# SebastianAment/CovarianceFunctions.jl

Hardware: AMD Instinct MI355X
Metric: Gramian MVMs/sec, dense EQ kernel, n=131072, d=3, fp32 (+ achieved HBM GB/s in roofline.hbm_*) (higher is better)
Workload: dtype f32; 1 GPU; EQ dense Gramian mul!, d=3 n=131072 fp32 (BASELINE.json configs[1]); x ~ N(0, I_3), a ~ N(0,1), alpha=1, beta=0, y == x; all n*m entries evaluated; points/a/b resident in HBM; n=131072, d=3, kernel=EQ, parallelism=1 GPU

## Files before the change

covariancefunctions.jl_amd/covgram/_ffi.py:

```python
from __future__ import annotations

import ctypes as C
import os

_HERE = os.path.dirname(os.path.abspath(__file__))
LIB_PATH = os.environ.get("COVGRAM_LIB") or os.path.normpath(os.path.join(_HERE, "..", "lib", "libcovgram.so"))

EQ, EXP, RQ, GAMMAEXP, CAUCHY, IMQ, MATERNP, DOT, EXPDOT, MATERN, ASINDOT = range(11)
CONSTANT, COMPOSITE = 100, 101
COMPOSITE_MAX_TERMS, COMPOSITE_MAX_FACTORS = 8, 8
ISOTROPIC, DOTPRODUCT = 1, 2
F32, F64 = 0, 1
HOST, DEVICE = 0, 1
OK, EINVAL, EUNSUPPORTED, EHIP, ENODEVICE, ENOMEM = 0, -1, -2, -3, -4, -5
MATERNP_MAX_P = 8
PIVCHOL_MAX_RANK = 1024
SM_MAX_COMPONENTS, SM_MAX_D = 32, 16
BILINEAR_MAX_NVEC, BILINEAR_MAX_D = 32, 64
COMM_ID_BYTES = 128
BCG_SLAB, BCG_FIELDS = 64, 8
BCG_RZ, BCG_TOL2, BCG_RR, BCG_ACTIVE, BCG_ITERS = range(5)
BLOCK_GRADIENT, BLOCK_VALUE_GRADIENT, BLOCK_HESSIAN, BLOCK_VALUE_GRADIENT_HESSIAN = range(4)
ABI_VERSION = 113

# ... 31 lines not shown

class DimensionMismatch(CovgramError, ValueError):
    """Julia's DimensionMismatch (src/util.jl:41, :9) — raised for COVGRAM_EINVAL."""


class UnsupportedKernel(CovgramError, NotImplementedError):
    """Kernel / dimension outside the compiled device set (COVGRAM_EUNSUPPORTED)."""


class NoDevice(CovgramError):
    """No gfx950 device: the product path fails loudly (COVGRAM_ENODEVICE)."""


_P = C.c_void_p
_I64 = C.c_int64
_I32 = C.c_int32
_D = C.c_double
_KP = C.POINTER(covgram_kernel)

PROTOTYPES = {
    "covgram_version": (C.c_int, []),
    "covgram_sizeof_kernel": (C.c_int, []),
    "covgram_sizeof_composite": (C.c_int, []),
    "covgram_last_error": (C.c_char_p, []),
    "covgram_device_count": (C.c_int, [C.POINTER(C.c_int)]),
    "covgram_ctx_create": (C.c_int, [C.POINTER(_P), C.c_int, _P]),
    "covgram_ctx_destroy": (C.c_int, [_P]),
    "covgram_ctx_set_stream": (C.c_int, [_P, _P]),
    "covgram_ctx_get_stream": (C.c_int, [_P, C.POINTER(_P)]),
    "covgram_ctx_set_option": (C.c_int, [_P, C.c_char_p, _I64]),
    "covgram_ctx_get_info": (C.c_int, [_P, C.c_char_p, C.POINTER(_I64)]),
    "covgram_sync": (C.c_int, [_P]),
    "covgram_ctx_kernel_time": (C.c_int, [_P, C.POINTER(_D), C.POINTER(_I64), _I32]),
    "covgram_points_create": (C.c_int, [_P, C.POINTER(_P), _P, _I64, _I32, _I32, _I32]),
    "covgram_points_slice": (C.c_int, [_P, _I64, _I64, C.POINTER(_P)]),
    "covgram_points_destroy": (C.c_int, [_P]),
    "covgram_points_info": (C.c_int, [_P, C.POINTER(_I64), C.POINTER(_I32), C.POINTER(_I32)]),
    "covgram_mvm": (C.c_int, [_P, _KP, _P, _P, _P, _I64, _P, _I64, _I32, _D, _D, _I32]),
    "covgram_matrix": (C.c_int, [_P, _KP, _P, _P, _P, _I64, _I32]),
    "covgram_grad_mvm": (C.c_int, [_P, _KP, _P, _P, _P, _I64, _P, _I64, _I32, _D, _D, _I32]),
    "covgram_valgrad_mvm": (C.c_int, [_P, _KP, _P, _P, _P, _I64, _P, _I64, _I32, _D, _D, _I32]),
    "covgram_hess_mvm": (C.c_int, [_P, _KP, _P, _P, _P, _I64, _P, _I64, _I32, _D, _D, _I32]),
    "covgram_valgradhess_mvm": (C.c_int, [_P, _KP, _P, _P, _P, _I64, _P, _I64, _I32, _D, _D, _I32]),
    "covgram_block_matrix": (C.c_int, [_P, _I32, _KP, _P, _P, _P, _I64, _I32]),
    "covgram_mvm_sym_supported": (C.c_int, [_P, _KP, _P, _I32, C.POINTER(C.c_int32)]),
    "covgram_mvm_sym_partial": (C.c_int, [_P, _KP, _P, _P, _P, _I32, _I32]),
    "covgram_comm_unique_id": (C.c_int, [_P, _I64]),
    "covgram_comm_create": (C.c_int, [_P, _P, _I32, _I32]),
    "covgram_comm_destroy": (C.c_int, [_P]),
    "covgram_comm_info": (C.c_int, [_P, C.POINTER(_I32), C.POINTER(_I32)]),
    "covgram_comm_all_gather": (C.c_int, [_P, _P, _P, _I64, _I32]),
    "covgram_comm_all_reduce_sum": (C.c_int, [_P, _P, _I64, _I32]),
    "covgram_mvm_sharded": (C.c_int, [_P, _KP, _P, _P, _P, _P, _D, _D]),
    "covgram_mvm_sym_allreduce": (C.c_int, [_P, _KP, _P, _P, _P, _D, _D]),
    "covgram_decay_radius": (C.c_int, [_KP, _D, C.POINTER(_D)]),
    "covgram_sparse_create": (C.c_int, [_P, C.POINTER(_P), _KP, _P, _P, _D]),
    "covgram_sparse_info": (C.c_int, [_P, C.POINTER(_I64), C.POINTER(_I64), C.POINTER(_I64), C.POINTER(_I32), C.POINTER(_D)]),
    "covgram_sparse_export": (C.c_int, [_P, _P, _P, _P, _I32]),
    "covgram_sparse_mvm": (C.c_int, [_P, _P, _I64, _P, _I64, _I32, _D, _D, _I32]),
    "covgram_sparse_destroy": (C.c_int, [_P]),
    "covgram_bh_create": (C.c_int, [_P, C.POINTER(_P), _KP, _P, _P, _D, _I32]),
    "covgram_bh_info": (C.c_int, [_P, C.POINTER(_I64), C.POINTER(_I64), C.POINTER(_I32), C.POINTER(_I32), C.POINTER(_I64), C.POINTER(_I32),
                                  C.POINTER(_D)]),
    "covgram_bh_export": (C.c_int, [_P, _P, _P, _P, _P, _P, _P, _P, _I32]),
    "covgram_bh_moments": (C.c_int, [_P, _P, _P, _P, _I32]),
    "covgram_bh_mvm": (C.c_int, [_P, _P, _P, _D, _D, _D, _I32, _P, _I64, _I32]),
# ... 64 lines not shown
```

covariancefunctions.jl_amd/csrc/api.hip:

```cpp
#include <math.h>
#include <stdarg.h>

#include <algorithm>
#include <vector>

#include "driver.hpp"
#include "dense_mvm.hpp"
#include "dense_sym32.hpp"
#include "dense_bcast.hpp"
#include "dense_wide.hpp"
#include "grad_wide.hpp"
#include "hess_mvm.hpp"
#include "block_matrix.hpp"

namespace covgram {

static thread_local char g_err[512] = "";

void set_error(const char* fmt, ...) {
    va_list ap;
    va_start(ap, fmt);
    vsnprintf(g_err, sizeof(g_err), fmt, ap);
    va_end(ap);
}
// ... 577 lines not shown
    ::covgram::DeviceGuard _cg_dev(ctx->device);
    (void)hipStreamSynchronize(ctx->stream);
    ctx_blas_destroy(ctx);
    (void)comm_destroy(ctx);
    for (auto& w : ctx->ws) if (w.ptr) (void)hipFree(w.ptr);
    if (ctx->sym_map) (void)hipFree(ctx->sym_map);
    if (ctx->stamp_buf) (void)hipFree(ctx->stamp_buf);
    if (ctx->tickets) (void)hipFree(ctx->tickets);
    for (auto& t : ctx->timers) { (void)hipEventDestroy(t.first); (void)hipEventDestroy(t.second); }
    if (ctx->own_stream) (void)hipStreamDestroy(ctx->stream);
    delete ctx;
    return COVGRAM_OK;
}

int covgram_ctx_set_stream(covgram_ctx* ctx, void* hip_stream) {
    CG_REQUIRE(ctx != nullptr, COVGRAM_EINVAL, "ctx is NULL");
    if ((hipStream_t)hip_stream != ctx->stream) CG_CHECK_HIP(hipStreamSynchronize(ctx->stream));
    ctx->stream = (hipStream_t)hip_stream;
    return COVGRAM_OK;
}

int covgram_ctx_get_stream(covgram_ctx* ctx, void** hip_stream) {
    CG_REQUIRE(ctx && hip_stream, COVGRAM_EINVAL, "NULL argument");
    *hip_stream = (void*)ctx->stream;
    return COVGRAM_OK;
}

struct CtxField { const char* key; int64_t covgram_ctx::*member; };
#define CG_FIELD(name) {#name, &covgram_ctx::name}
static const CtxField kOptions[] = {
    CG_FIELD(dense_variant), CG_FIELD(toeplitz_fused), CG_FIELD(toeplitz_colfft), CG_FIELD(toeplitz_persist), CG_FIELD(kron_fill), CG_FIELD(mfma_f16),
    CG_FIELD(mfma_gate_pct), CG_FIELD(mfma_fuse_w), CG_FIELD(toeplitz_real_spectrum), CG_FIELD(rows_per_lane), CG_FIELD(jsplit), CG_FIELD(target_wgs),
    CG_FIELD(grad_keep_r), CG_FIELD(grad_expand), CG_FIELD(grad_bcast), CG_FIELD(mfma_lds), CG_FIELD(mfma_sym), CG_FIELD(dense_sym), CG_FIELD(dense_bcast),
    CG_FIELD(mfma_stamp), CG_FIELD(inkernel_reduce), CG_FIELD(matrix_variant), CG_FIELD(mfma_mrhs), CG_FIELD(composite_termwise), CG_FIELD(sum_fused),
    CG_FIELD(lowrank_reverse), CG_FIELD(mfma_sym_rt), CG_FIELD(mfma_sym_st), CG_FIELD(lowrank_wgs), CG_FIELD(time_kernels)};
static const CtxField kInfo[] = {
    CG_FIELD(last_dense_path), CG_FIELD(last_jsplit), CG_FIELD(last_kron_path), CG_FIELD(last_mfma_lds), CG_FIELD(last_mfma_sym), CG_FIELD(last_dense_sym),
    CG_FIELD(last_dense_bcast), CG_FIELD(last_mfma_f16), CG_FIELD(last_inkernel_reduce), CG_FIELD(last_grad_expand), CG_FIELD(last_grad_bcast),
    CG_FIELD(last_grad_path), CG_FIELD(last_grad_jsplit), CG_FIELD(last_hess_path), CG_FIELD(last_vgh_path), CG_FIELD(last_matrix_path),
    CG_FIELD(last_block_matrix_path), CG_FIELD(last_sum_fused), CG_FIELD(last_mfma_instance), CG_FIELD(last_mfma_sym_rt), CG_FIELD(num_cus)};
#undef CG_FIELD

int covgram_ctx_set_option(covgram_ctx* ctx, const char* key, int64_t value) {
    CG_REQUIRE(ctx && key, COVGRAM_EINVAL, "NULL argument");
    for (const CtxField& f : kOptions) {
        if (strcmp(key, f.key)) continue;
        if (!strcmp(key, "mfma_gate_pct")) CG_REQUIRE(value >= 1 && value <= 100, COVGRAM_EINVAL, "mfma_gate_pct = %lld: 1..100", (long long)value);
        if (!strcmp(key, "time_kernels")) ctx->timers_used = 0;
        ctx->*f.member = value;
        return COVGRAM_OK;
    }
    set_error("unknown option '%s'", key);
    return COVGRAM_EINVAL;
}

int covgram_ctx_get_info(covgram_ctx* ctx, const char* key, int64_t* value) {
    CG_REQUIRE(ctx && key && value, COVGRAM_EINVAL, "NULL argument");
    for (const CtxField& f : kInfo)
        if (!strcmp(key, f.key)) { *value = ctx->*f.member; return COVGRAM_OK; }
    if (!strcmp(key, "last_clock_khz")) {
        *value = 0;
        if (ctx->stamp_count > 0 && ctx->stamp_buf) {
            CG_DEVICE(ctx);
            CG_CHECK_HIP(hipStreamSynchronize(ctx->stream));
            std::vector<unsigned long long> h(ctx->stamp_count * 4);
            CG_CHECK_HIP(hipMemcpy(h.data(), ctx->stamp_buf, h.size() * sizeof(unsigned long long), hipMemcpyDeviceToHost));
            std::vector<double> khz;
            for (size_t w = 0; w < ctx->stamp_count; ++w) {
                const double dc = (double)(h[4 * w + 2] - h[4 * w]), dr = (double)(h[4 * w + 3] - h[4 * w + 1]);
                if (h[4 * w + 3] > h[4 * w + 1] && dr >= 100.0) khz.push_back(dc / dr * 1.0e5);
            }
            if (!khz.empty()) { std::nth_element(khz.begin(), khz.begin() + khz.size() / 2, khz.end()); *value = (int64_t)khz[khz.size() / 2]; }
        }
        return COVGRAM_OK;
    }
    set_error("unknown info key '%s'", key);
    return COVGRAM_EINVAL;
}

int covgram_ctx_kernel_time(covgram_ctx* ctx, double* total_ms, int64_t* launches, int32_t reset) {
    CG_REQUIRE(ctx && total_ms && launches, COVGRAM_EINVAL, "NULL argument");
    CG_CHECK_HIP(hipStreamSynchronize(ctx->stream));
    double tot = 0;
    for (size_t i = 0; i < ctx->timers_used; ++i) {
        float ms = 0;
        CG_CHECK_HIP(hipEventElapsedTime(&ms, ctx->timers[i].first, ctx->timers[i].second));
        tot += ms;
    }
    *total_ms = tot;
    *launches = (int64_t)ctx->timers_used;
    if (reset) ctx->timers_used = 0;
    return COVGRAM_OK;
}

int covgram_sync(covgram_ctx* ctx) {
    CG_REQUIRE(ctx != nullptr, COVGRAM_EINVAL, "ctx is NULL");
    CG_CHECK_HIP(hipStreamSynchronize(ctx->stream));
    return COVGRAM_OK;
}

int covgram_points_create(covgram_ctx* ctx, covgram_points** out, const void* x, int64_t n, int32_t d, int32_t dtype,
                          int32_t loc) {
    CG_REQUIRE(ctx && out, COVGRAM_EINVAL, "NULL argument");
    CG_REQUIRE(n >= 0 && d >= 1, COVGRAM_EINVAL, "points: need n >= 0 and d >= 1 (got n=%lld d=%d)", (long long)n, d);
    CG_REQUIRE(dtype == COVGRAM_F32 || dtype == COVGRAM_F64, COVGRAM_EINVAL, "unknown dtype %d", dtype);
    CG_REQUIRE(x != nullptr || n == 0, COVGRAM_EINVAL, "points pointer is NULL");
    CG_DEVICE(ctx);
    covgram_points* p = new covgram_points();
    p->ctx = ctx; p->n = n; p->d = d; p->dtype = dtype;
    if (loc == COVGRAM_DEVICE) { p->dptr = const_cast<void*>(x); p->owns = false; }
// ... 107 lines not shown
```

covariancefunctions.jl_amd/csrc/common.hpp:

```cpp
#pragma once
#include <hip/hip_runtime.h>
#include <math.h>
#include <stdint.h>
#include <stdio.h>
#include <stdlib.h>
#include <string.h>

#include <string>
#include <utility>
#include <vector>

#include "../../include/covgram.h"

namespace covgram {

__device__ __forceinline__ float fma_t(float a, float b, float c) { return __builtin_fmaf(a, b, c); }
__device__ __forceinline__ double fma_t(double a, double b, double c) { return __builtin_fma(a, b, c); }


void set_error(const char* fmt, ...);

#define CG_CHECK_HIP(expr)                                                                          \
    do {                                                                                            \
        hipError_t _e = (expr);                                                                     \
// ... 185 lines not shown
}

struct covgram_ctx {
    int device = 0;
    hipStream_t stream = nullptr;
    bool own_stream = false;
    covgram::Workspace ws[6];
    int64_t dense_variant = 0;
    int64_t rows_per_lane = 0;
    int64_t jsplit = 0;
    int64_t target_wgs = 0;
    int64_t grad_expand = -1;
    int64_t grad_keep_r = -1;
    int64_t grad_bcast = -1;
    int64_t last_grad_bcast = 0;
    int64_t mfma_sym_rt = -1;
    int64_t last_mfma_sym_rt = 0;
    int64_t mfma_sym_st = 0;
    int64_t lowrank_wgs = 0;
    int64_t lowrank_reverse = -1;
    int64_t sum_fused = -1;
    int64_t last_sum_fused = 0;
    int64_t composite_termwise = 1;
    int64_t dense_sym = -1;
    int64_t last_dense_sym = 0;
    int64_t dense_bcast = -1;
    int64_t last_dense_bcast = 0;
    int64_t inkernel_reduce = -1;
    int64_t last_inkernel_reduce = 0;
    unsigned* tickets = nullptr;
    size_t tickets_cap = 0;
    int64_t mfma_sym = -1;
    int64_t mfma_lds = -1;
    int64_t mfma_stamp = 0;
    void* stamp_buf = nullptr;
    size_t stamp_cap = 0, stamp_count = 0;
    int64_t matrix_variant = 0;
    int64_t mfma_mrhs = -1;
    int64_t toeplitz_real_spectrum = 1;
    int64_t toeplitz_colfft = 16;
    int64_t mfma_fuse_w = -1;
    int64_t kron_fill = 1;
    int64_t mfma_gate_pct = 100;
    int64_t mfma_f16 = -1;
    int64_t last_mfma_f16 = 0;
    int64_t last_mfma_instance = 0;
    int64_t toeplitz_persist = -1;
    int64_t toeplitz_fused = 1;
    void* comm = nullptr;
    int32_t comm_rank = 0, comm_world = 0;
    int64_t num_cus = 256;
    void* blas = nullptr;
    int live_handles = 0;
    int64_t last_dense_path = 0;
    int64_t last_kron_path = 0;
    int64_t last_jsplit = 0;
    int32_t* sym_map = nullptr;
    size_t sym_map_cap = 0, sym_map_len = 0;
    int64_t sym_key[4] = {-1, -1, -1, -1};
    int64_t last_mfma_sym = 0;
    int64_t last_grad_expand = 0;
    int64_t last_grad_path = 0;
    int64_t last_grad_jsplit = 0;
    int64_t last_hess_path = 0;
    int64_t last_matrix_path = 0;
    int64_t last_vgh_path = 0;
// ... 48 lines not shown
    int32_t sym = 0; void* colslab = nullptr;
    int32_t sym_first = 0, sym_stride = 1;
    double alpha, beta;
    const HostKernel* hk;
    hipStream_t stream;
};
typedef int (*dense_launch_fn)(const DenseArgs&, int dtype);
dense_launch_fn dense_launcher(int family);
dense_launch_fn dense_wide_launcher(int family);

struct GradArgs {
    const void* X; int64_t n; int32_t d;
    const void* P; int64_t m;
    void* out; int64_t npad;
    int32_t Dpad; int64_t jchunk; int32_t jsplit;
    int32_t keep_r;
    const void* C = nullptr;
    int32_t vg = 0;
    const void* A0 = nullptr;
    double alpha0 = 0, vg_c = 0, vg_b = 0;
    int32_t nr = 1;
    int64_t ldy = 0;
    int32_t expd = 0;
    const void* Ex = nullptr;
    int32_t bcast = 0;
    double alpha, beta;
    const HostKernel* hk;
    hipStream_t stream;
};
typedef int (*grad_launch_fn)(const GradArgs&, int dtype);
grad_launch_fn grad_launcher(int family);

constexpr int MFMA_LDS_MIN_TILES = 64;
constexpr int64_t MFMA_SYM_MIN_N_EQ = 18000;
constexpr int64_t MFMA_SYM_MIN_N_EQ_WIDE = 15000;
constexpr int64_t MFMA_SYM_MIN_N_HEAVY = 12500;
constexpr double MFMA_GATE = 126.0;
constexpr double MFMA_F16_GATE = 72.0;
inline double mfma_gate_of(const covgram_ctx* ctx) { return MFMA_GATE * 0.01 * (double)ctx->mfma_gate_pct; }
inline double mfma_f16_gate_of(const covgram_ctx* ctx) { return MFMA_F16_GATE * 0.01 * (double)ctx->mfma_gate_pct; }
constexpr double GRAD_EXPAND_GATE_F32 = 128.0;
constexpr double GRAD_EXPAND_GATE = 1000.0;
double gate_radius2(const covgram_points* X, const covgram_points* Y);
int points_max_norm2(covgram_points* p);
bool mfma_eq_eligible(const covgram_ctx* ctx, const HostKernel& hk, const covgram_points* X, const covgram_points* Y, int nrhs);
int mvm_eq_mfma(covgram_ctx* ctx, const HostKernel& hk, const covgram_points* X, const covgram_points* Y, const float* a, float* y,
                double alpha, double beta);
bool mfma_eq_sym_eligible(const covgram_ctx* ctx, const HostKernel& hk, const covgram_points* X, const covgram_points* Y, int nrhs);
int mvm_eq_mfma_sym(covgram_ctx* ctx, const HostKernel& hk, const covgram_points* X, const float* a, float* y, double alpha, double beta,
                    int pfirst = 0, int pstride = 1, const covgram_kernel* kgen = nullptr);
bool mfma_gen_sym_eligible(const covgram_ctx* ctx, const HostKernel& hk, const covgram_points* X, const covgram_points* Y, int nrhs);
bool mfma_gen_eligible(const covgram_ctx* ctx, const HostKernel& hk, const covgram_points* X, const covgram_points* Y, int nrhs = 1);
bool sum_fused_applies(const covgram_ctx* ctx, const covgram_kernel* k, const covgram_points* X, const covgram_points* Y, int nrhs);
int mvm_mfma_gen(covgram_ctx* ctx, const covgram_kernel* k, const covgram_points* X, const covgram_points* Y, const float* a, int64_t lda,
                 float* y, int64_t ldy, int32_t nrhs, double alpha, double beta);

int mvm_dot_factored(covgram_ctx* ctx, const HostKernel& hk, const covgram_points* X, const covgram_points* Y, const void* a, int64_t lda, void* y,
                     int64_t ldy, int32_t nrhs, double alpha, double beta);

void ctx_blas_destroy(covgram_ctx* ctx);
int comm_destroy(covgram_ctx* ctx);

int pad_dim(int d);
extern const int kDims[];
extern const int kNumDims;

// ... 2 lines not shown
```

covariancefunctions.jl_amd/csrc/dense_mfma.hip:

```cpp
#include "driver.hpp"
#include "mfma_plan.hpp"
#include "dense_mfma_eq.hpp"

namespace covgram {

template <typename T, int DL = 1>
__global__ __launch_bounds__(256) void max_norm2_kernel(const T* __restrict__ X, int64_t n, int32_t d, unsigned* __restrict__ outbits,
                                                        const T* __restrict__ Cn) {
    float v = 0.0f, vc = 0.0f;
    const int64_t g0 = (int64_t)blockIdx.x * blockDim.x + threadIdx.x, gs = (int64_t)gridDim.x * blockDim.x;
    const int cl = (int)(g0 % DL);
    for (int64_t i = g0 / DL; i < (n + 63) / 64 * 64; i += gs / DL) {
        double s = 0, sc = 0;
        if constexpr (DL == 1) {
            if (i >= n) continue;
            for (int c = 0; c < d; ++c) {
                const double xc = (double)X[i * (int64_t)d + c], xd = xc - (double)Cn[c];
                s += xc * xc; sc += xd * xd;
            }
        } else {
            if (i < n) { const double xc = (double)X[i * (int64_t)DL + cl], xd = xc - (double)Cn[cl]; s = xc * xc; sc = xd * xd; }
#pragma unroll
            for (int o = DL / 2; o > 0; o >>= 1) { s += __shfl_xor(s, o); sc += __shfl_xor(sc, o); }
        }
        float f = (float)s, fc = (float)sc;
        if (!(f >= 0.0f)) f = __builtin_inff();
        if (!(fc >= 0.0f)) fc = __builtin_inff();
        v = fmaxf(v, f * 1.000001f);
        vc = fmaxf(vc, fc * 1.000001f);
    }
#pragma unroll
    for (int o = 32; o > 0; o >>= 1) { v = fmaxf(v, __shfl_xor(v, o)); vc = fmaxf(vc, __shfl_xor(vc, o)); }
    __shared__ float wmax[4], wcmax[4];
    if ((threadIdx.x & 63) == 0) { wmax[threadIdx.x >> 6] = v; wcmax[threadIdx.x >> 6] = vc; }
    __syncthreads();
    if (threadIdx.x == 0) {
        atomicMax(outbits, __float_as_uint(fmaxf(fmaxf(wmax[0], wmax[1]), fmaxf(wmax[2], wmax[3]))));
// ... 226 lines not shown
    return pl.js == 1 ? COVGRAM_OK : ws_reserve(ctx, 1, (size_t)pl.js * nrpad * pl.npad * sizeof(float), (void**)out);
}
static void reduce_split(covgram_ctx* ctx, const float* slab, const ColumnPlan& pl, int nrpad, float* y, int64_t n, int64_t ldy, int nr, double alpha,
                         double beta) {
    hipLaunchKernelGGL(dense_reduce_kernel<float>, dim3((unsigned)((n + 63) / 64), nr), dim3(256), 0, ctx->stream, slab, pl.npad, nrpad, (int)pl.js, y, n,
                       ldy, nr, (float)alpha, (float)beta);
}

static int gen_fragments(covgram_ctx* ctx, const covgram_points* Y, const float* a, int64_t lda, int nr, int NR, int K2, float gam, bool iso, int fmt,
                         size_t extra, const uint4** PB, float** W) {
    const int64_t ntile = (Y->n + 31) / 32, pe = ntile * K2 * 64;
    void* P;
    int rc = ws_reserve(ctx, 0, (size_t)ntile * ((size_t)K2 * 64 * sizeof(uint4) + (size_t)NR * 32 * sizeof(float)) + extra, &P);
    if (rc) return rc;
    *PB = (const uint4*)P;
    *W = (float*)((uint4*)P + pe);
    hipLaunchKernelGGL(mfma_pack_gen_kernel, dim3((unsigned)((pe + 255) / 256)), dim3(256), 0, ctx->stream, (const float*)Y->dptr, Y->n, Y->d, a, lda, nr, 0,
                       (uint4*)P, *W, K2, NR, gam, iso ? 1 : 0, (const float*)Y->center, fmt);
    return COVGRAM_OK;
}

template <int K2, int RT>
static int mfma_blocks_per_cu() {
    static int cached = 0;
    if (!cached) {
        int nb = 0;
        if (hipOccupancyMaxActiveBlocksPerMultiprocessor(&nb, dense_mfma_eq_kernel<K2, RT>, 64, 0) != hipSuccess || nb <= 0) nb = 16;
        cached = nb;
    }
    return cached;
}
template <int K2, int RT, int WPB, int LDS, int STAMP, int FMT>
static void eq_launch(covgram_ctx* ctx, const MfmaArgs& a, dim3* launched) {
    ctx->last_mfma_instance = (int64_t)K2 * 100000 + RT * 10000 + WPB * 1000 + LDS * 100 + STAMP * 10 + FMT;
    *launched = dim3((a.grid.x + WPB - 1) / WPB, a.grid.y);
    hipLaunchKernelGGL((dense_mfma_eq_kernel<K2, RT, WPB, LDS, STAMP, FMT>), *launched, dim3(64 * WPB), 0, a.stream, a.X, a.n, a.d, a.PB, a.W, a.ntile, a.out,
                       a.npad, a.tchunk, a.g, a.alpha, a.beta, a.final_store, a.Cn, STAMP ? a.stamps : nullptr, a.tickets, a.yfinal, a.EF, a.mcols);
}
template <int K2, int FMT>
static void eq_launch_instance(covgram_ctx* ctx, const MfmaArgs& a, dim3* launched) {
    constexpr bool NARROW = K2 <= MFMA_NARROW_MAXK2;
    const bool stamp = a.stamps != nullptr;
    if (a.lds) {
        if constexpr (K2 <= 2) {
            if (a.grid.x >= 1024) return stamp ? eq_launch<K2, 2, 8, 1, 1, FMT>(ctx, a, launched) : eq_launch<K2, 2, 8, 1, 0, FMT>(ctx, a, launched);
        }
        if constexpr (K2 == 3 || K2 == 4) { if (a.RT == 4) return eq_launch<K2, 4, 4, 1, 0, FMT>(ctx, a, launched); }
        if constexpr (K2 == 1 || K2 == 2 || K2 == 4) { if (stamp) return eq_launch<K2, 2, 4, 1, 1, FMT>(ctx, a, launched); }
        constexpr int LDSF = (NARROW || K2 == 6) ? 1 : 2;
        return eq_launch<K2, (NARROW ? 2 : 1), 4, LDSF, 0, FMT>(ctx, a, launched);
    }
    if constexpr (K2 <= 8) { if (a.RT == 2) return eq_launch<K2, 2, 1, 0, 0, FMT>(ctx, a, launched); }
    eq_launch<K2, 1, 1, 0, 0, FMT>(ctx, a, launched);
}

static int eq_fragments(covgram_ctx* ctx, const covgram_points* Y, int K2, float g, const float* Cn, const uint4** PB, const float** EF, int fmt = 0) {
    const int64_t m = Y->n, ntile = (m + 31) / 32;
    const size_t fbytes = (size_t)ntile * K2 * 64 * sizeof(uint4);
    const size_t total = fbytes + (size_t)ntile * 32 * sizeof(float);
    covgram_points::FragSlot* hit = nullptr;
    covgram_points::FragSlot* victim = nullptr;
    hipStreamCaptureStatus cs = hipStreamCaptureStatusNone;
    const bool capturing = ctx->stream && hipStreamIsCapturing(ctx->stream, &cs) == hipSuccess && cs != hipStreamCaptureStatusNone;
    for (auto& f : Y->frag) {
        if (f.ptr && f.bytes == total && f.g == g && f.k2 == K2 && f.fmt == fmt) { hit = &f; break; }
        if (f.pinned) continue;
        const auto rank = [&](const covgram_points::FragSlot& s) { return !s.ptr ? 0 : (s.bytes != total ? 1 : 2); };
        if (!victim || rank(f) < rank(*victim) || (rank(f) == rank(*victim) && f.used < victim->used)) victim = &f;
    }
    if (!hit) {
// ... 40 lines not shown
    if (rc) return rc;
    const bool overlap = (const char*)a < (const char*)(y + n) && (const char*)y < (const char*)(a + m);
    const bool fuse_w = ctx->mfma_fuse_w != 0 && !overlap;
    ma.W = a; ma.EF = EF;
    if (!fuse_w) {
        void* Wp;
        rc = ws_reserve(ctx, 0, (size_t)ntile * 32 * sizeof(float), &Wp);
        if (rc) return rc;
        hipLaunchKernelGGL(mfma_pack_w_kernel, dim3((unsigned)((ntile * 32 + 255) / 256)), dim3(256), 0, ctx->stream, a, EF, (float*)Wp, m, ntile * 32);
        ma.W = (const float*)Wp; ma.EF = nullptr;
    }
    int rt = ctx->rows_per_lane == 1 ? 1 : (ctx->rows_per_lane == 2 ? 2 : (K2 <= MFMA_NARROW_MAXK2 ? 2 : 1));
    if (K2 > 8) rt = 1;
    int nb = 16;
    mfma_for_k2(K2, [&](auto k) {
        constexpr int K = decltype(k)::value;
        if constexpr (K <= 8) { if (rt == 2) { nb = mfma_blocks_per_cu<K, 2>(); return; } }
        nb = mfma_blocks_per_cu<K, 1>();
    });
    struct Plan { ColumnPlan col; int rt; bool lds4; };
    auto plan_for = [&](int r) {
        Plan pl; pl.rt = r;
        const int64_t target = ctx->target_wgs > 0 ? ctx->target_wgs : (int64_t)ctx->num_cus * nb * 4;
        pl.col = plan_columns(n, ntile, 32 * r, target, ctx->jsplit, 8, 64, 2048, 16);
        pl.lds4 = ((r >= 2 && K2 <= MFMA_NARROW_MAXK2) || (r == 1 && K2 > MFMA_NARROW_MAXK2)) &&
                  (ctx->mfma_lds == 1 || (ctx->mfma_lds < 0 && pl.col.tchunk >= MFMA_LDS_MIN_TILES && pl.col.rowtiles >= 64));
        return pl;
    };
    Plan pl = plan_for(rt);
    if ((K2 == 3 || K2 == 4) && pl.lds4 && pl.rt == 2 && (ctx->rows_per_lane == 4 || (ctx->rows_per_lane == 0 && K2 == 4 && !ctx->mfma_stamp))) {
        const Plan p4 = plan_for(4);
        if (p4.lds4) pl = p4;
    }
    const ColumnPlan& col = pl.col;
    ma.RT = pl.rt; ma.lds = pl.lds4 ? 1 : 0;
    ma.npad = col.npad; ma.tchunk = col.tchunk; ma.final_store = col.js == 1 ? 1 : 0;
    ma.grid = dim3((unsigned)col.rowtiles, (unsigned)col.js);
    rc = split_out(ctx, col, 1, y, &ma.out);
    if (rc) return rc;
    ctx->stamp_count = 0;
    if (ctx->mfma_stamp && pl.lds4 && (K2 == 1 || K2 == 2 || K2 == 4)) {
        const size_t need = (size_t)col.rowtiles * col.js * 4 * sizeof(unsigned long long);
        if (need > ctx->stamp_cap) {
            if (ctx->stamp_buf) { CG_CHECK_HIP(hipStreamSynchronize(ctx->stream)); (void)hipFree(ctx->stamp_buf); ctx->stamp_buf = nullptr; ctx->stamp_cap = 0; }
            CG_CHECK_HIP(hipMalloc(&ctx->stamp_buf, need));
            ctx->stamp_cap = need;
        }
        CG_CHECK_HIP(hipMemsetAsync(ctx->stamp_buf, 0, need, ctx->stream));
        ma.stamps = (unsigned long long*)ctx->stamp_buf;
    }
    const bool ikr = inkernel_reduce_on(ctx, true, n, col.js);
    ctx->last_inkernel_reduce = ikr ? 1 : 0;
    if (ikr) { rc = tickets_reserve(ctx, (size_t)col.rowtiles, &ma.tickets); if (rc) return rc; }
    ctx->last_mfma_lds = ma.lds;
    dim3 launched;
    {
        TimerScope tm(ctx);
        const bool compiled = mfma_for_k2(K2, [&](auto k) {
            constexpr int K = decltype(k)::value;
            if (!fmt) eq_launch_instance<K, 0>(ctx, ma, &launched);
            else if constexpr (K <= 8) eq_launch_instance<K, 1>(ctx, ma, &launched);
        });
        CG_REQUIRE(compiled, COVGRAM_EUNSUPPORTED, "dense_mfma: K2 = %d not compiled", K2);
    }
    if (ma.stamps) ctx->stamp_count = (size_t)launched.x * launched.y;
    if (col.js > 1 && !ikr) reduce_split(ctx, ma.out, col, 1, y, n, n, 1, alpha * hk.kp.scale, beta);
    hipError_t e = hipGetLastError();
    if (e != hipSuccess) { set_error("dense_mfma launch failed: %s", hipGetErrorString(e)); return COVGRAM_EHIP; }
    return COVGRAM_OK;
}
// ... 240 lines not shown
```

covariancefunctions.jl_amd/csrc/dense_mfma.hpp:

```cpp
#pragma once
#include "dense_mvm.hpp"
#include <type_traits>

namespace covgram {

typedef float f32x16 __attribute__((ext_vector_type(16)));
typedef __bf16 bf16x8 __attribute__((ext_vector_type(8)));
typedef unsigned short u16x8 __attribute__((ext_vector_type(8)));

__device__ __forceinline__ unsigned bf16_bits(float f) {
    unsigned u = __float_as_uint(f);
    u += 0x7FFFu + ((u >> 16) & 1u);
    return u >> 16;
}
__device__ __forceinline__ void split3(float f, unsigned& p1, unsigned& p2, unsigned& p3) {
    p1 = bf16_bits(f);
    const float r1 = f - __uint_as_float(p1 << 16);
    p2 = bf16_bits(r1);
    const float r2 = r1 - __uint_as_float(p2 << 16);
    p3 = bf16_bits(r2);
}

typedef _Float16 f16x8 __attribute__((ext_vector_type(8)));
union Frag {
// ... 869 lines not shown
        CG_TILE2(ti, tfA, twA, csA)
        if (wv == 0 && h == 0) twB[t] = CG_GW;
        __syncthreads();
        if (ti + 1 >= nt) { CG_FLUSH2(ti, csA) break; }
        CG_DMA2(ti + 2, tfA)
        CG_FLUSH2(ti, csA)
        CG_TILE2(ti + 1, tfB, twB, csB)
        if (wv == 0 && h == 0) twA[t] = CG_GW;
        __syncthreads();
        if (ti + 2 >= nt) { CG_FLUSH2(ti + 1, csB) }
    }
#undef CG_DMA2
#undef CG_TILE2
#undef CG_FLUSH2
#undef CG_GW

    const int vsel = (t & 3) + 4 * (t >> 3);
    float tot = 0.0f;
#pragma unroll
    for (int v = 0; v < 16; ++v) {
        float s = acc[v];
        s += __shfl_xor(s, 1); s += __shfl_xor(s, 2); s += __shfl_xor(s, 4); s += __shfl_xor(s, 8); s += __shfl_xor(s, 16);
        tot = (vsel == v) ? s : tot;
    }
    const int64_t i = i0 + t;
    if (((t >> 2) & 1) != h || i >= n) return;
    R[cabs * npad + i] = FAST ? er * tot : tot;
}

}
#include "dense_mfma_sym2.hpp"
namespace covgram {

struct MfmaArgs {
    const float* X; int64_t n; int32_t d;
    const uint4* PB; const float* W; int64_t ntile;
    float* out; int64_t npad; int64_t ldy; int32_t nrhs;
    int64_t tchunk; float alpha, beta; int32_t final_store;
    int32_t K2, RT, NR;
    const HostKernel* hk;
    hipStream_t stream;
    dim3 grid;
    const float* Cn = nullptr;
    int32_t fmt = 0;
    int32_t lds = 0;
    int32_t mrhs = 0;
    int32_t sym = 0;
    int32_t sym_rt = 1;
    float* R = nullptr; float* S = nullptr;
    const int32_t* wgmap = nullptr;
    int32_t pfirst = 0, pstride = 1;
    float g = 0.0f; const float* EF = nullptr; int64_t mcols = 0;
    unsigned* tickets = nullptr; float* yfinal = nullptr; unsigned long long* stamps = nullptr;
};

template <int FAM, int K2, int RT, int NR, int ORD, int GFMT>
static void mfma_gen_launch_f(const MfmaArgs& a) {
    auto go = [&](auto lds, dim3 grid, int block) {
        hipLaunchKernelGGL((dense_mfma_gen_kernel<FAM, K2, RT, NR, decltype(lds)::value, ORD, GFMT>), grid, dim3(block), 0, a.stream, a.X, a.n, a.d, a.PB, a.W, a.ntile,
                           a.out, a.npad, a.ldy, a.nrhs, a.tchunk, a.alpha, a.beta, a.final_store, a.Cn, make_params<FAM, float>(*a.hk));
    };
    if (a.lds) go(std::integral_constant<int, 2>{}, dim3((a.grid.x + 3) / 4, a.grid.y), 256);
    else go(std::integral_constant<int, 0>{}, a.grid, 64);
}
template <int FAM, int K2, int NB>
static int mfma_mrhs_one(const MfmaArgs& a) {
    hipLaunchKernelGGL((dense_mfma_mrhs_kernel<FAM, K2, NB>), a.grid, dim3(64), 0, a.stream, a.X, a.n, a.d, a.PB, a.W, a.ntile, a.out, a.npad,
                       a.ldy, a.nrhs, a.tchunk, a.alpha, a.beta, a.final_store, a.Cn, make_params<FAM, float>(*a.hk));
    return COVGRAM_OK;
}
template <auto Kernel, int BLOCK, typename KP>
static void mfma_sym_launch(const MfmaArgs& a, const KP& kp) {
    hipLaunchKernelGGL(Kernel, a.grid, dim3(BLOCK), 0, a.stream, a.X, a.n, a.d, a.PB, a.W, a.ntile, a.R, a.S, a.npad, (int32_t)a.tchunk, a.g, a.Cn,
                       a.pfirst, a.pstride, a.wgmap, kp, a.EF);
}

template <int FAM, int K2> constexpr bool mfma_gen_has_f16 = fam_is_iso<FAM> && !fam_is_expr<FAM> && K2 <= 8;
template <int FAM, int K2, int RT, int NR, int ORD>
static void mfma_gen_launch(const MfmaArgs& a) {
    if constexpr (mfma_gen_has_f16<FAM, K2>) { if (a.fmt == 1) { mfma_gen_launch_f<FAM, K2, RT, NR, ORD, 1>(a); return; } }
    mfma_gen_launch_f<FAM, K2, RT, NR, ORD, 0>(a);
}
template <int FAM, int K2, int RT, int NR>
static int mfma_gen_one(const MfmaArgs& a, bool query) {
    if (query) {
        static int cached = 0;
// ... 93 lines not shown
```

covariancefunctions.jl_amd/csrc/dense_mfma_eq.hpp:

```cpp
#pragma once
#include "dense_mfma.hpp"

namespace covgram {

__global__ __launch_bounds__(256) void mfma_pack_kernel(const float* __restrict__ Y, int64_t m, int32_t d, uint4* __restrict__ PB,
                                                        float* __restrict__ EF, int32_t K2, float g, const float* __restrict__ Cn, int32_t fmt) {
    const int64_t e = (int64_t)blockIdx.x * blockDim.x + threadIdx.x;
    const int64_t ntile = (m + 31) / 32;
    if (e >= ntile * K2 * 64) return;
    const int l = (int)(e & 63);
    const int64_t q = e >> 6;
    const int mm = (int)(q % K2);
    const int64_t T = q / K2;
    const int64_t j = 32 * T + (l & 31);
    if (fmt == 1) {
        const int c0 = 4 * mm + 2 * (l >> 5);
        const bool nl = mm == 0 && (l >> 5) == 0;
        uint4 frag = make_uint4(0, 0, 0, 0);
        if (j < m) {
            const float ya = c0 < d ? g * (Y[j * (int64_t)d + c0] - Cn[c0]) : 0.0f;
            const float yb = c0 + 1 < d ? g * (Y[j * (int64_t)d + c0 + 1] - Cn[c0 + 1]) : 0.0f;
            unsigned a1, a2, b1, b2;
            split2h(ya, a1, a2);
            split2h(yb, b1, b2);
// ... 17 lines not shown
    if (j < m) {
        if (c < d) {
            const float yt = g * (Y[j * (int64_t)d + c] - Cn[c]);
            unsigned y1, y2, y3;
            split3(yt, y1, y2, y3);
            frag = make_uint4(y1 | (y2 << 16), y1 | (y3 << 16), y2 | (y1 << 16), y3 | (y2 << 16));
        }
        if (norm_lane) {
            double ny = 0.0;
            for (int cc = 0; cc < d; ++cc) { const double yc = (double)(g * (Y[j * (int64_t)d + cc] - Cn[cc])); ny = __builtin_fma(yc, yc, ny); }
            const NormSplit sp = norm_split(ny);
            if (d & 1) frag = make_uint4(BF16_ONE | (sp.kbits << 16), 0, 0, 0);
            else frag.w = BF16_ONE | (sp.kbits << 16);
            EF[j] = sp.ef;
        }
    } else if (norm_lane) {
        EF[j] = 0.0f;
    }
    PB[e] = frag;
}

__global__ __launch_bounds__(256) void mfma_pack_w_kernel(const float* __restrict__ A, const float* __restrict__ EF, float* __restrict__ W,
                                                          int64_t m, int64_t mpad) {
    const int64_t j = (int64_t)blockIdx.x * blockDim.x + threadIdx.x;
    if (j < mpad) W[j] = j < m ? A[j] * EF[j] : 0.0f;
}

template <int K2, int RT, int WPB = 1, int LDS = 0, int STAMP = 0, int FMT = 0>
__global__ __launch_bounds__(64 * WPB) __attribute__((amdgpu_waves_per_eu(LDS == 1 ? (RT == 4 ? 2 : K2 <= 2 ? 4 : 3) : 1, LDS == 1 ? (RT == 4 ? 2 : K2 <= 2 ? 4 : 3) : 8))) void dense_mfma_eq_kernel(const float* __restrict__ X, int64_t n, int32_t d,
                                                           const uint4* __restrict__ PB, const float* __restrict__ W, int64_t ntile,
                                                           float* __restrict__ out, int64_t npad, int64_t tchunk, float g,
                                                           float alpha, float beta, int32_t final_store, const float* __restrict__ Cn,
                                                           unsigned long long* __restrict__ stamps, unsigned* __restrict__ tickets,
                                                           float* __restrict__ yfinal, const float* __restrict__ EF, int64_t mcols) {
    const int l = threadIdx.x & 63, t = l & 31, h = l >> 5;
    const int64_t i0 = ((int64_t)blockIdx.x * WPB + (threadIdx.x >> 6)) * (32 * RT);
    Frag a[RT][K2];
    float er[RT];
#pragma unroll
    for (int r = 0; r < RT; ++r) {
        int64_t row = i0 + 32 * r + t;
        if (row >= n) row = n - 1;
        er[r] = eq_row_fragments_fmt<K2, FMT>(X + row * (int64_t)d, Cn, d, g, h, a[r]);
    }

    unsigned long long st_c0 = 0, st_r0 = 0;
    if constexpr (STAMP) { st_c0 = __builtin_amdgcn_s_memtime(); st_r0 = __builtin_amdgcn_s_memrealtime(); }
    const int64_t T0 = (int64_t)blockIdx.y * tchunk;
    const int64_t T1 = (T0 + tchunk < ntile) ? (T0 + tchunk) : ntile;
    typedef float f32x2 __attribute__((ext_vector_type(2)));
    f32x2 acc2[RT][8];
#pragma unroll
    for (int r = 0; r < RT; ++r)
#pragma unroll
        for (int v = 0; v < 8; ++v) acc2[r][v] = (f32x2){0.0f, 0.0f};

    const uint4* __restrict__ pbase = PB + (T0 * K2) * 64;
    const float* __restrict__ wbase = W + T0 * 32;
    const int nt = (int)(T1 - T0);
    auto weight = [&](int tc) {
        if (EF == nullptr) return wbase[tc * 32 + t];
        const int64_t j = (T0 + tc) * 32 + t;
        return j < mcols ? W[j] * EF[j] : 0.0f;
    };
    auto load_tile = [&](int ti, Frag (&f)[K2], float& w) {
        const int tc = ti < nt ? ti : nt - 1;
#pragma unroll
        for (int mm = 0; mm < K2; ++mm) f[mm].u = pbase[(tc * K2 + mm) * 64 + l];
        w = weight(tc);
    };
    auto process = [&](const Frag (&f)[K2], float w) {
        f32x16 D[RT];
#pragma unroll
        for (int r = 0; r < RT; ++r) {
            D[r] = (f32x16){0, 0, 0, 0, 0, 0, 0, 0, 0, 0, 0, 0, 0, 0, 0, 0};
#pragma unroll
            for (int mm = 0; mm < K2; ++mm) D[r] = eq_mma<FMT>(a[r][mm], f[mm], D[r]);
        }
#pragma unroll
        for (int r = 0; r < RT; ++r)
#pragma unroll
            for (int v = 0; v < 16; ++v) D[r][v] = __builtin_amdgcn_exp2f(D[r][v]);
// ... 222 lines not shown
```

covariancefunctions.jl_amd/csrc/mfma_plan.hpp:

```cpp
#pragma once
#include <algorithm>
#include <cstdint>
#include <vector>

namespace covgram {

struct ColumnPlan { int64_t rowtiles, npad, js, tchunk; };

inline ColumnPlan plan_columns(int64_t n, int64_t ntile, int rows, int64_t target, int64_t jsplit, int64_t min_tiles, int64_t stop_tiles = 0,
                               int64_t floor_waves = 0, int64_t floor_tiles = 1) {
    ColumnPlan pl;
    pl.rowtiles = (n + rows - 1) / rows;
    pl.npad = pl.rowtiles * rows;
    int64_t js = jsplit > 0 ? jsplit : std::max<int64_t>(1, (target + pl.rowtiles / 2) / pl.rowtiles);
    if (jsplit <= 0 && stop_tiles > 0)
        js = std::max<int64_t>(std::min<int64_t>((floor_waves + pl.rowtiles - 1) / pl.rowtiles, std::max<int64_t>(1, ntile / floor_tiles)),
                               std::min<int64_t>(js, std::max<int64_t>(1, ntile / stop_tiles)));
    js = std::max<int64_t>(1, std::min<int64_t>(js, std::max<int64_t>(1, ntile / min_tiles)));
    pl.tchunk = (ntile + js - 1) / js;
    pl.js = (ntile + pl.tchunk - 1) / pl.tchunk;
    return pl;
}

constexpr int SYM_CHUNK_BITS = 12, SYM_PANEL_BITS = 19;
inline int64_t sym_panels(int64_t ntile, int tpp) { return (ntile + tpp - 1) / tpp; }
inline int64_t sym_local_panels(int64_t ntile, int tpp, int64_t pfirst, int64_t pstride) {
    const int64_t panels = sym_panels(ntile, tpp);
    return panels > pfirst ? (panels - pfirst + pstride - 1) / pstride : 0;
}
inline int64_t sym_chunks(int64_t ntile, int64_t tchunk) { return (ntile + tchunk - 1) / tchunk; }
inline bool sym_list_in_range(int64_t ntile, int tpp, int64_t tchunk, int64_t pfirst, int64_t pstride) {
    return sym_chunks(ntile, tchunk) <= ((int64_t)1 << SYM_CHUNK_BITS) && sym_local_panels(ntile, tpp, pfirst, pstride) < ((int64_t)1 << SYM_PANEL_BITS);
}

inline std::vector<int32_t> sym_worklist(int64_t ntile, int tpp, int64_t tchunk, int64_t pfirst, int64_t pstride) {
    const int64_t maxc = sym_chunks(ntile, tchunk), lpanels = sym_local_panels(ntile, tpp, pfirst, pstride);
    const auto len = [&](int64_t lp, int64_t c) {
        return std::min((c + 1) * tchunk, ntile) - std::max(c * tchunk, tpp * (pfirst + pstride * lp));
    };
    std::vector<int32_t> list, tail;
    for (int64_t c = 0; c < maxc; ++c)
        for (int64_t lp = 0; lp < lpanels && len(lp, c) > 0; ++lp)
            (len(lp, c) == tchunk ? list : tail).push_back((int32_t)((lp << SYM_CHUNK_BITS) | c));
    std::sort(tail.begin(), tail.end(), [&](int32_t u, int32_t v) {
        const int64_t lu = len(u >> SYM_CHUNK_BITS, u & ((1 << SYM_CHUNK_BITS) - 1)), lv = len(v >> SYM_CHUNK_BITS, v & ((1 << SYM_CHUNK_BITS) - 1));
        return lu != lv ? lu > lv : u < v;
    });
    list.insert(list.end(), tail.begin(), tail.end());
    return list;
}

}
```

include/covgram.h:

```cpp
#ifndef COVGRAM_H
#define COVGRAM_H

#include <stdint.h>

#ifdef __cplusplus
extern "C" {
#endif

#define COVGRAM_VERSION 113

typedef enum covgram_status {
    COVGRAM_OK = 0,
    COVGRAM_EINVAL = -1,
    COVGRAM_EUNSUPPORTED = -2,
    COVGRAM_EHIP = -3,
    COVGRAM_ENODEVICE = -4,
    COVGRAM_ENOMEM = -5
} covgram_status;

typedef enum covgram_family {
    COVGRAM_EQ = 0,
    COVGRAM_EXP = 1,
    COVGRAM_RQ = 2,
    COVGRAM_GAMMAEXP = 3,
// ... 25 lines not shown
    double lengthscale;
    double scale;
} covgram_kernel;

#define COVGRAM_COMPOSITE_MAX_TERMS 8
#define COVGRAM_COMPOSITE_MAX_FACTORS 8
typedef struct covgram_kernel_composite {
    covgram_kernel head;
    int32_t nterms;
    int32_t nfactors[COVGRAM_COMPOSITE_MAX_TERMS];
    covgram_kernel factors[COVGRAM_COMPOSITE_MAX_FACTORS];
} covgram_kernel_composite;

typedef struct covgram_ctx covgram_ctx;
typedef struct covgram_points covgram_points;
typedef struct covgram_toeplitz covgram_toeplitz;
typedef struct covgram_sparse covgram_sparse;
typedef struct covgram_bh covgram_bh;

int covgram_version(void);
int covgram_sizeof_kernel(void);
int covgram_sizeof_composite(void);
const char* covgram_last_error(void);
int covgram_device_count(int* count);

int covgram_ctx_create(covgram_ctx** ctx, int device_id, void* hip_stream);
int covgram_ctx_destroy(covgram_ctx* ctx);
int covgram_ctx_set_stream(covgram_ctx* ctx, void* hip_stream);
int covgram_ctx_get_stream(covgram_ctx* ctx, void** hip_stream);
int covgram_ctx_set_option(covgram_ctx* ctx, const char* key, int64_t value);
int covgram_ctx_get_info(covgram_ctx* ctx, const char* key, int64_t* value);
int covgram_sync(covgram_ctx* ctx);
int covgram_ctx_kernel_time(covgram_ctx* ctx, double* total_ms, int64_t* launches, int32_t reset);

int covgram_points_create(covgram_ctx* ctx, covgram_points** out, const void* x, int64_t n, int32_t d,
                          int32_t dtype, int32_t loc);
int covgram_points_slice(const covgram_points* parent, int64_t first, int64_t count, covgram_points** out);
int covgram_points_destroy(covgram_points* pts);
int covgram_points_info(const covgram_points* pts, int64_t* n, int32_t* d, int32_t* dtype);

int covgram_mvm(covgram_ctx* ctx, const covgram_kernel* k, const covgram_points* X, const covgram_points* Y,
                const void* a, int64_t lda, void* y, int64_t ldy, int32_t nrhs, double alpha, double beta,
                int32_t loc);

int covgram_matrix(covgram_ctx* ctx, const covgram_kernel* k, const covgram_points* X, const covgram_points* Y,
                   void* out, int64_t ldo, int32_t loc);

int covgram_mvm_sym_supported(covgram_ctx* ctx, const covgram_kernel* k, const covgram_points* X, int32_t world, int32_t* supported);
int covgram_mvm_sym_partial(covgram_ctx* ctx, const covgram_kernel* k, const covgram_points* X, const void* a, void* y,
                            int32_t rank, int32_t world);

#define COVGRAM_COMM_ID_BYTES 128
int covgram_comm_unique_id(void* id, int64_t bytes);
int covgram_comm_create(covgram_ctx* ctx, const void* unique_id, int32_t rank, int32_t world);
int covgram_comm_destroy(covgram_ctx* ctx);
int covgram_comm_info(const covgram_ctx* ctx, int32_t* rank, int32_t* world);
int covgram_comm_all_gather(covgram_ctx* ctx, const void* send, void* recv, int64_t count, int32_t dtype);
int covgram_comm_all_reduce_sum(covgram_ctx* ctx, void* buf, int64_t count, int32_t dtype);
int covgram_mvm_sharded(covgram_ctx* ctx, const covgram_kernel* k, const covgram_points* X, const covgram_points* Y, const void* a,
                        void* y, double alpha, double beta);
int covgram_mvm_sym_allreduce(covgram_ctx* ctx, const covgram_kernel* k, const covgram_points* X, const void* a, void* y, double alpha,
                              double beta);

int covgram_grad_mvm(covgram_ctx* ctx, const covgram_kernel* k, const covgram_points* X, const covgram_points* Y, const void* a,
                     int64_t lda, void* y, int64_t ldy, int32_t nrhs, double alpha, double beta, int32_t loc);

// ... 108 lines not shown
```

Baseline: 733.7 MVM/s.

## Grade MFMA column chunk sizes to shrink the tail wave

```diff
diff --git a/covariancefunctions.jl_amd/covgram/_ffi.py b/covariancefunctions.jl_amd/covgram/_ffi.py
--- a/covariancefunctions.jl_amd/covgram/_ffi.py
+++ b/covariancefunctions.jl_amd/covgram/_ffi.py
@@ -87,6 +87,7 @@
     "covgram_ctx_get_info": (C.c_int, [_P, C.c_char_p, C.POINTER(_I64)]),
     "covgram_sync": (C.c_int, [_P]),
     "covgram_ctx_kernel_time": (C.c_int, [_P, C.POINTER(_D), C.POINTER(_I64), _I32]),
+    "covgram_ctx_read_stamps": (C.c_int, [_P, C.POINTER(C.c_uint64), _I64, C.POINTER(_I64)]),
     "covgram_points_create": (C.c_int, [_P, C.POINTER(_P), _P, _I64, _I32, _I32, _I32]),
     "covgram_points_slice": (C.c_int, [_P, _I64, _I64, C.POINTER(_P)]),
     "covgram_points_destroy": (C.c_int, [_P]),
diff --git a/covariancefunctions.jl_amd/csrc/api.hip b/covariancefunctions.jl_amd/csrc/api.hip
--- a/covariancefunctions.jl_amd/csrc/api.hip
+++ b/covariancefunctions.jl_amd/csrc/api.hip
@@ -633,13 +633,13 @@
     CG_FIELD(dense_variant), CG_FIELD(toeplitz_fused), CG_FIELD(toeplitz_colfft), CG_FIELD(toeplitz_persist), CG_FIELD(kron_fill), CG_FIELD(mfma_f16),
     CG_FIELD(mfma_gate_pct), CG_FIELD(mfma_fuse_w), CG_FIELD(toeplitz_real_spectrum), CG_FIELD(rows_per_lane), CG_FIELD(jsplit), CG_FIELD(target_wgs),
     CG_FIELD(grad_keep_r), CG_FIELD(grad_expand), CG_FIELD(grad_bcast), CG_FIELD(mfma_lds), CG_FIELD(mfma_sym), CG_FIELD(dense_sym), CG_FIELD(dense_bcast),
-    CG_FIELD(mfma_stamp), CG_FIELD(inkernel_reduce), CG_FIELD(matrix_variant), CG_FIELD(mfma_mrhs), CG_FIELD(composite_termwise), CG_FIELD(sum_fused),
+    CG_FIELD(mfma_stamp), CG_FIELD(mfma_graded), CG_FIELD(inkernel_reduce), CG_FIELD(matrix_variant), CG_FIELD(mfma_mrhs), CG_FIELD(composite_termwise), CG_FIELD(sum_fused),
     CG_FIELD(lowrank_reverse), CG_FIELD(mfma_sym_rt), CG_FIELD(mfma_sym_st), CG_FIELD(lowrank_wgs), CG_FIELD(time_kernels)};
 static const CtxField kInfo[] = {
     CG_FIELD(last_dense_path), CG_FIELD(last_jsplit), CG_FIELD(last_kron_path), CG_FIELD(last_mfma_lds), CG_FIELD(last_mfma_sym), CG_FIELD(last_dense_sym),
     CG_FIELD(last_dense_bcast), CG_FIELD(last_mfma_f16), CG_FIELD(last_inkernel_reduce), CG_FIELD(last_grad_expand), CG_FIELD(last_grad_bcast),
     CG_FIELD(last_grad_path), CG_FIELD(last_grad_jsplit), CG_FIELD(last_hess_path), CG_FIELD(last_vgh_path), CG_FIELD(last_matrix_path),
-    CG_FIELD(last_block_matrix_path), CG_FIELD(last_sum_fused), CG_FIELD(last_mfma_instance), CG_FIELD(last_mfma_sym_rt), CG_FIELD(num_cus)};
+    CG_FIELD(last_block_matrix_path), CG_FIELD(last_sum_fused), CG_FIELD(last_mfma_instance), CG_FIELD(last_mfma_graded), CG_FIELD(last_mfma_sym_rt), CG_FIELD(num_cus)};
 #undef CG_FIELD
 
 int covgram_ctx_set_option(covgram_ctx* ctx, const char* key, int64_t value) {
@@ -677,6 +677,17 @@
     }
     set_error("unknown info key '%s'", key);
     return COVGRAM_EINVAL;
+}
+
+int covgram_ctx_read_stamps(covgram_ctx* ctx, uint64_t* out, int64_t cap, int64_t* count) {
+    CG_REQUIRE(ctx && count && cap >= 0 && (out || cap == 0), COVGRAM_EINVAL, "NULL argument");
+    *count = ctx->stamp_buf ? (int64_t)ctx->stamp_count : 0;
+    const size_t take = (size_t)std::min<int64_t>(*count, cap);
+    if (take == 0) return COVGRAM_OK;
+    CG_DEVICE(ctx);
+    CG_CHECK_HIP(hipStreamSynchronize(ctx->stream));
+    CG_CHECK_HIP(hipMemcpy(out, ctx->stamp_buf, take * 4 * sizeof(uint64_t), hipMemcpyDeviceToHost));
+    return COVGRAM_OK;
 }
 
 int covgram_ctx_kernel_time(covgram_ctx* ctx, double* total_ms, int64_t* launches, int32_t reset) {
diff --git a/covariancefunctions.jl_amd/csrc/common.hpp b/covariancefunctions.jl_amd/csrc/common.hpp
--- a/covariancefunctions.jl_amd/csrc/common.hpp
+++ b/covariancefunctions.jl_amd/csrc/common.hpp
@@ -241,6 +241,8 @@
     size_t tickets_cap = 0;
     int64_t mfma_sym = -1;
     int64_t mfma_lds = -1;
+    int64_t mfma_graded = -1;
+    int64_t last_mfma_graded = 0;
     int64_t mfma_stamp = 0;
     void* stamp_buf = nullptr;
     size_t stamp_cap = 0, stamp_count = 0;
@@ -355,6 +357,7 @@
 grad_launch_fn grad_launcher(int family);
 
 constexpr int MFMA_LDS_MIN_TILES = 64;
+constexpr int MFMA_GRADED_TAIL_HALFROUNDS = 1;
 constexpr int64_t MFMA_SYM_MIN_N_EQ = 18000;
 constexpr int64_t MFMA_SYM_MIN_N_EQ_WIDE = 15000;
 constexpr int64_t MFMA_SYM_MIN_N_HEAVY = 12500;
diff --git a/covariancefunctions.jl_amd/csrc/dense_mfma.hip b/covariancefunctions.jl_amd/csrc/dense_mfma.hip
--- a/covariancefunctions.jl_amd/csrc/dense_mfma.hip
+++ b/covariancefunctions.jl_amd/csrc/dense_mfma.hip
@@ -3,6 +3,7 @@
 #include "dense_mfma_eq.hpp"
 
 namespace covgram {
+static_assert(GRADED_MAX_CHUNKS == MFMA_MAX_CHUNKS, "the planner's table and the kernel argument hold the same number of chunks");
 
 template <typename T, int DL = 1>
 __global__ __launch_bounds__(256) void max_norm2_kernel(const T* __restrict__ X, int64_t n, int32_t d, unsigned* __restrict__ outbits,
@@ -295,10 +296,20 @@
 }
 template <int K2, int RT, int WPB, int LDS, int STAMP, int FMT>
 static void eq_launch(covgram_ctx* ctx, const MfmaArgs& a, dim3* launched) {
+    *launched = dim3((a.grid.x + WPB - 1) / WPB, a.grid.y);
+    if (a.occupancy) {
+        static int cached = 0;
+        if (!cached) {
+            int nb = 0;
+            if (hipOccupancyMaxActiveBlocksPerMultiprocessor(&nb, dense_mfma_eq_kernel<K2, RT, WPB, LDS, STAMP, FMT>, 64 * WPB, 0) != hipSuccess || nb <= 0) nb = std::max(1, 16 / WPB);
+            cached = nb;
+        }
+        a.occupancy[0] = cached; a.occupancy[1] = WPB;
+        return;
+    }
     ctx->last_mfma_instance = (int64_t)K2 * 100000 + RT * 10000 + WPB * 1000 + LDS * 100 + STAMP * 10 + FMT;
-    *launched = dim3((a.grid.x + WPB - 1) / WPB, a.grid.y);
     hipLaunchKernelGGL((dense_mfma_eq_kernel<K2, RT, WPB, LDS, STAMP, FMT>), *launched, dim3(64 * WPB), 0, a.stream, a.X, a.n, a.d, a.PB, a.W, a.ntile, a.out,
-                       a.npad, a.tchunk, a.g, a.alpha, a.beta, a.final_store, a.Cn, STAMP ? a.stamps : nullptr, a.tickets, a.yfinal, a.EF, a.mcols);
+                       a.npad, a.tchunk, a.g, a.alpha, a.beta, a.final_store, a.Cn, STAMP ? a.stamps : nullptr, a.tickets, a.yfinal, a.EF, a.mcols, a.chunks);
 }
 template <int K2, int FMT>
 static void eq_launch_instance(covgram_ctx* ctx, const MfmaArgs& a, dim3* launched) {
@@ -405,10 +416,39 @@
         const Plan p4 = plan_for(4);
         if (p4.lds4) pl = p4;
     }
-    const ColumnPlan& col = pl.col;
+    ColumnPlan col = pl.col;
     ma.RT = pl.rt; ma.lds = pl.lds4 ? 1 : 0;
+    ma.grid = dim3((unsigned)col.rowtiles, (unsigned)col.js);
+    ctx->last_mfma_graded = 0;
+    if (ctx->mfma_graded != 0 && ctx->jsplit <= 0 && ctx->target_wgs <= 0 && col.js > 1) {
+        const bool lds_shape = ((pl.rt >= 2 && K2 <= MFMA_NARROW_MAXK2) || (pl.rt == 1 && K2 > MFMA_NARROW_MAXK2)) && col.tchunk >= MFMA_LDS_MIN_TILES &&
+                               col.rowtiles >= 64;
+        int occ[2] = {0, 1};
+        dim3 unused;
+        MfmaArgs q = ma;
+        q.lds = lds_shape ? 1 : ma.lds; q.occupancy = occ;
+        mfma_for_k2(K2, [&](auto k) {
+            constexpr int K = decltype(k)::value;
+            if (!fmt) eq_launch_instance<K, 0>(ctx, q, &unused);
+            else if constexpr (K <= 8) eq_launch_instance<K, 1>(ctx, q, &unused);
+        });
+        const bool force = ctx->mfma_graded > 0;
+        const int64_t wpb = occ[1], rblocks = (col.rowtiles + wpb - 1) / wpb, slots = (int64_t)ctx->num_cus * occ[0];
+        const bool clamped = plan_columns(n, ntile, 32 * pl.rt, (int64_t)ctx->num_cus * nb * 4, 0, 8).js != col.js;
+        int64_t floor_tiles = col.tchunk >= 2 * MFMA_LDS_MIN_TILES ? MFMA_LDS_MIN_TILES : 8, halfrounds = MFMA_GRADED_TAIL_HALFROUNDS;
+        if (ctx->mfma_graded >= 100) { halfrounds = ctx->mfma_graded / 100; floor_tiles = (int64_t)16 << (ctx->mfma_graded % 10); }
+        if (force || (lds_shape && !clamped)) {
+            const GradedPlan gp = plan_columns_graded(col, ntile, rblocks, slots, q.lds ? wpb : 2 , floor_tiles, force, halfrounds);
+            if (gp.graded) {
+                col.js = gp.js;
+                ma.chunks.n = (int32_t)gp.js;
+                for (int c = 0; c <= GRADED_MAX_CHUNKS; ++c) ma.chunks.start[c] = gp.start[c];
+                ma.grid.y = (unsigned)gp.js;
+                ctx->last_mfma_graded = gp.js;
+            }
+        }
+    }
     ma.npad = col.npad; ma.tchunk = col.tchunk; ma.final_store = col.js == 1 ? 1 : 0;
-    ma.grid = dim3((unsigned)col.rowtiles, (unsigned)col.js);
     rc = split_out(ctx, col, 1, y, &ma.out);
     if (rc) return rc;
     ctx->stamp_count = 0;
diff --git a/covariancefunctions.jl_amd/csrc/dense_mfma.hpp b/covariancefunctions.jl_amd/csrc/dense_mfma.hpp
--- a/covariancefunctions.jl_amd/csrc/dense_mfma.hpp
+++ b/covariancefunctions.jl_amd/csrc/dense_mfma.hpp
@@ -925,6 +925,9 @@
 #include "dense_mfma_sym2.hpp"
 namespace covgram {
 
+constexpr int MFMA_MAX_CHUNKS = 64;
+struct ChunkTable { int32_t n = 0; int32_t start[MFMA_MAX_CHUNKS + 1] = {}; };
+
 struct MfmaArgs {
     const float* X; int64_t n; int32_t d;
     const uint4* PB; const float* W; int64_t ntile;
@@ -945,6 +948,8 @@
     int32_t pfirst = 0, pstride = 1;
     float g = 0.0f; const float* EF = nullptr; int64_t mcols = 0;
     unsigned* tickets = nullptr; float* yfinal = nullptr; unsigned long long* stamps = nullptr;
+    ChunkTable chunks;
+    int* occupancy = nullptr;
 };
 
 template <int FAM, int K2, int RT, int NR, int ORD, int GFMT>
diff --git a/covariancefunctions.jl_amd/csrc/dense_mfma_eq.hpp b/covariancefunctions.jl_amd/csrc/dense_mfma_eq.hpp
--- a/covariancefunctions.jl_amd/csrc/dense_mfma_eq.hpp
+++ b/covariancefunctions.jl_amd/csrc/dense_mfma_eq.hpp
@@ -73,7 +73,8 @@
                                                            float* __restrict__ out, int64_t npad, int64_t tchunk, float g,
                                                            float alpha, float beta, int32_t final_store, const float* __restrict__ Cn,
                                                            unsigned long long* __restrict__ stamps, unsigned* __restrict__ tickets,
-                                                           float* __restrict__ yfinal, const float* __restrict__ EF, int64_t mcols) {
+                                                           float* __restrict__ yfinal, const float* __restrict__ EF, int64_t mcols,
+                                                           const ChunkTable chunks) {
     const int l = threadIdx.x & 63, t = l & 31, h = l >> 5;
     const int64_t i0 = ((int64_t)blockIdx.x * WPB + (threadIdx.x >> 6)) * (32 * RT);
     Frag a[RT][K2];
@@ -87,8 +88,9 @@
 
     unsigned long long st_c0 = 0, st_r0 = 0;
     if constexpr (STAMP) { st_c0 = __builtin_amdgcn_s_memtime(); st_r0 = __builtin_amdgcn_s_memrealtime(); }
-    const int64_t T0 = (int64_t)blockIdx.y * tchunk;
-    const int64_t T1 = (T0 + tchunk < ntile) ? (T0 + tchunk) : ntile;
+    int64_t T0 = (int64_t)blockIdx.y * tchunk;
+    int64_t T1 = (T0 + tchunk < ntile) ? (T0 + tchunk) : ntile;
+    if (chunks.n > 0) { T0 = chunks.start[blockIdx.y]; T1 = chunks.start[blockIdx.y + 1]; }
     typedef float f32x2 __attribute__((ext_vector_type(2)));
     f32x2 acc2[RT][8];
 #pragma unroll
diff --git a/covariancefunctions.jl_amd/csrc/mfma_plan.hpp b/covariancefunctions.jl_amd/csrc/mfma_plan.hpp
--- a/covariancefunctions.jl_amd/csrc/mfma_plan.hpp
+++ b/covariancefunctions.jl_amd/csrc/mfma_plan.hpp
@@ -20,6 +20,44 @@
     pl.tchunk = (ntile + js - 1) / js;
     pl.js = (ntile + pl.tchunk - 1) / pl.tchunk;
     return pl;
+}
+
+constexpr int GRADED_MAX_CHUNKS = 64;
+struct GradedPlan { bool graded; int64_t js; int32_t start[GRADED_MAX_CHUNKS + 1]; };
+
+inline GradedPlan plan_columns_graded(const ColumnPlan& base, int64_t ntile, int64_t rblocks, int64_t slots, int64_t stage, int64_t floor_tiles,
+                                      bool force, int64_t tail_halfrounds = 2) {
+    GradedPlan g;
+    g.graded = false; g.js = base.js;
+    for (int64_t c = 0; c <= GRADED_MAX_CHUNKS; ++c) g.start[c] = (int32_t)std::min<int64_t>(c * base.tchunk, ntile);
+    if (base.js < 2 || rblocks < 1 || slots < 1 || stage < 1 || ntile > INT32_MAX) return g;
+    if (!force && (rblocks * base.js < 2 * slots || base.tchunk < floor_tiles)) return g;
+    const int64_t tail_chunks = std::max<int64_t>(1, std::min<int64_t>((tail_halfrounds * slots + rblocks) / (2 * rblocks), base.js / 2));
+    const int64_t body = base.js - tail_chunks;
+    for (int64_t floor = (std::max<int64_t>(floor_tiles, 1) + stage - 1) / stage * stage;; floor *= 2) {
+        int64_t len = base.tchunk / 2 / stage * stage;
+        if (len < floor || body > GRADED_MAX_CHUNKS) return g;
+        int64_t js = body, at = body * base.tchunk, left = ntile - at;
+        int32_t start[GRADED_MAX_CHUNKS + 1];
+        for (int64_t c = 0; c <= body; ++c) start[c] = (int32_t)(c * base.tchunk);
+        bool fits = true;
+        while (left > 0 && fits) {
+            int64_t k = len > floor ? std::min<int64_t>((left / 2 + len - 1) / len, left / len) : left / len;
+            if (len == floor && k == 0) k = 1;
+            for (; k > 0 && fits; --k) {
+                const int64_t take = std::min(len, left);
+                if (js >= GRADED_MAX_CHUNKS) { fits = false; break; }
+                at += take; left -= take; start[++js] = (int32_t)at;
+            }
+            if (len > floor) len = std::max(floor, len / 2 / stage * stage);
+            else if (left > 0 && left < len) len = left;
+        }
+        if (!fits) continue;
+        g.graded = true; g.js = js;
+        for (int64_t c = 0; c <= js; ++c) g.start[c] = start[c];
+        for (int64_t c = js + 1; c <= GRADED_MAX_CHUNKS; ++c) g.start[c] = (int32_t)ntile;
+        return g;
+    }
 }
 
 constexpr int SYM_CHUNK_BITS = 12, SYM_PANEL_BITS = 19;
diff --git a/include/covgram.h b/include/covgram.h
--- a/include/covgram.h
+++ b/include/covgram.h
@@ -81,6 +81,7 @@
 int covgram_ctx_get_info(covgram_ctx* ctx, const char* key, int64_t* value);
 int covgram_sync(covgram_ctx* ctx);
 int covgram_ctx_kernel_time(covgram_ctx* ctx, double* total_ms, int64_t* launches, int32_t reset);
+int covgram_ctx_read_stamps(covgram_ctx* ctx, uint64_t* out, int64_t cap, int64_t* count);
 
 int covgram_points_create(covgram_ctx* ctx, covgram_points** out, const void* x, int64_t n, int32_t d,
                           int32_t dtype, int32_t loc);
```

Measured after the change: 741.6 MVM/s (median of 6 runs). 1.1% higher.
